# XuyangBai/D3Feat.pytorch

Hardware: AMD Instinct MI355X
Metric: fragment-pairs/sec (fwd+bwd) on 3DMatch-shaped pairs (higher is better)
Workload: dtype f32

## Files before the change

### d3feat.pytorch_amd/csrc/kpconv_dx_gather.hip

```cpp
#include "kpconv_tile.hpp"

namespace d3f {

void* kpconv_timing_open(int which, hipStream_t stream, int Nq, int Ns, int H, int Cin, int Cout, int K);
void kpconv_timing_close(void* rec, hipStream_t stream);

struct RevTest {
  const uint64_t* last_key;
  float sx, sy, sz;
  unsigned s;
  float r2;
};

template <int CV, bool HAS_NN>
__device__ __forceinline__ void dxg_table_chunk(int n, float qx, float qy, float qz, float nnv, uint64_t lk,
                                                const RevTest& rt, int Nq, int last_lane, int32_t* status,
                                                float4* scr4, float* scr1, __amdgpu_buffer_rsrc_t rs_g,
                                                unsigned row_bytes, unsigned col_off, float cx, float cy, float cz,
                                                float inv_extent, int lane, int lg, f32x4 (&acc)[CV]) {
  const float d2 = sqdist_exact(qx, qy, qz, rt.sx, rt.sy, rt.sz);
  const uint64_t key = ((uint64_t)__float_as_uint(d2) << 32) | rt.s;
  const bool in_r = rt.r2 <= 0.0f || d2 < rt.r2;
  const bool member = n < Nq && key <= lk && in_r;
  if (rt.r2 > 0.0f && status && lane == last_lane && n < Nq && d2 < rt.r2) atomicOr(status, D3F_ST_WIDE_OVERFLOW);
  const uint64_t m = __ballot(member);
  const int cnt = __popcll(m);
  if (cnt == 0) return;
  const int rank = __popcll(m & ((1ull << lane) - 1ull));
  if (member) {
    scr4[rank] = make_float4(qx - rt.sx, qy - rt.sy, qz - rt.sz, __int_as_float(n));
    scr1[rank] = HAS_NN ? 1.0f / nnv : 1.0f;
  }
  __builtin_amdgcn_fence(__ATOMIC_RELEASE, "wavefront");
  __builtin_amdgcn_wave_barrier();
  const bool mine = lane < cnt;
  const float4 c = scr4[mine ? lane : 0];
  const float inn = mine ? scr1[lane] : 0.0f;
  const int n_c = mine ? __float_as_int(c.w) : Nq;
  __builtin_amdgcn_wave_barrier();
  dxg_core_n<CV>((cnt + 15) >> 4, n_c, c.x, c.y, c.z, inn, rs_g, row_bytes, col_off, cx, cy, cz, inv_extent, lg, acc);
}

template <int CV, int NBW, int WK, bool HAS_NN>
__global__ __launch_bounds__(256) void kpconv_dx_gather_kernel(
    const float* __restrict__ s_pts, const float* __restrict__ q_pts, const int32_t* __restrict__ rev_ptr,
    const int32_t* __restrict__ rev_ent, const float* __restrict__ gout, const float* __restrict__ nn,
    const float* __restrict__ kp, const float* __restrict__ W, int Ns, int Nq, int Cin, int Cout, int K, float extent,
    float* __restrict__ gx, const uint64_t* __restrict__ last_key, int rev_width, float rev_r2,
    int32_t* __restrict__ status, unsigned long long* __restrict__ clk, const float4* __restrict__ rev_rel) {
  PhaseClock pc;
  pc.start(clk);
  constexpr int CC = 16 * CV;
  constexpr int WN = 4 / WK;
  extern __shared__ __attribute__((aligned(16))) float lds[];
  constexpr int RS = 16 * CC + 4;
  float* tile = lds;
  float4* scr4 = (float4*)(lds + 16 * RS) + (threadIdx.x >> 6) * 64;
  float* scr1 = lds + 16 * RS + 4 * 256 + (threadIdx.x >> 6) * 64;
  float* red = lds + 16 * RS + 5 * 256;

  const int lane = threadIdx.x & 63, wave = threadIdx.x >> 6;
  const int li = lane & 15, lg = lane >> 4;
  const int s0 = blockIdx.x * 16;
  float kx, ky, kz;
  load_kernel_point(kp, K, li, kx, ky, kz);
  const __amdgpu_buffer_rsrc_t rs_q = make_rsrc(q_pts, (unsigned)Nq * 12u);
  const __amdgpu_buffer_rsrc_t rs_nn = make_rsrc(HAS_NN ? nn : q_pts, (unsigned)Nq * 4u);
  const __amdgpu_buffer_rsrc_t rs_g = make_rsrc(gout, (unsigned)Nq * (unsigned)Cout * 4u);
  const float inv_extent = 1.0f / extent;
  const int wn = (WK == 1) ? wave : (WK == 2 ? (wave & 1) : 0);
  const int wk = (WK == 1) ? 0 : (WK == 2 ? (wave >> 1) : wave);
  constexpr int SLAB = 16 * NBW * WN;
  const int n_base = blockIdx.y * SLAB;

  constexpr int NACC = NBW == 1 ? 2 : 1;
  f32x4 acc2[NBW][NACC];
#pragma unroll
  for (int nb = 0; nb < NBW; ++nb)
#pragma unroll
    for (int a = 0; a < NACC; ++a) acc2[nb][a] = (f32x4){0.f, 0.f, 0.f, 0.f};
  if (WK > 1)
    for (int t = threadIdx.x; t < 16 * SLAB; t += 256) red[t] = 0.0f;

  const unsigned row_bytes = (unsigned)Cout * 4u;
  const int nchunks = Cout / CC;
  pc.lap(0);
  for (int ch = 0; ch < nchunks; ++ch) {
    const int cbase = ch * CC;
    const unsigned col_off = (unsigned)(cbase + li * CV) * 4u;
    if (rev_rel) {
      const int W = rev_width;
      float4 eA[4];
#pragma unroll
      for (int i = 0; i < 4; ++i) {
        const int s = s0 + wave * 4 + i;
        eA[i] = rev_rel[(size_t)min(s, Ns - 1) * W + min(lane, W - 1)];
        if (!(s < Ns && lane < W)) eA[i].w = __int_as_float(Nq);
      }
      if (clk) {
        asm volatile("s_waitcnt vmcnt(0)" ::: "memory");
        pc.lap(1);
      }
#pragma unroll 1
      for (int i = 0; i < 4; ++i) {
        const int s = s0 + wave * 4 + i;
        f32x4 acc[CV];
#pragma unroll
        for (int r = 0; r < CV; ++r) acc[r] = (f32x4){0.f, 0.f, 0.f, 0.f};
        if (s < Ns) {
          float4 e = eA[0];
          for (int c0 = 0; c0 < W; c0 += 64) {
            if (c0 > 0) {
              e = rev_rel[(size_t)s * W + min(c0 + lane, W - 1)];
              if (c0 + lane >= W) e.w = __int_as_float(Nq);
            }
            const int n = min(max(__float_as_int(e.w), 0), Nq);
            const int cnt = __popcll(__ballot(n < Nq));
            if (cnt == 0) break;
            if (HAS_NN)
              dxg_core_n<CV, true>((cnt + 15) >> 4, n, e.x, e.y, e.z, 0.0f, rs_g, row_bytes, col_off, -kx, -ky, -kz,
                                   inv_extent, lg, acc, Nq, rs_nn);
            else
              dxg_core_n<CV>((cnt + 15) >> 4, n, e.x, e.y, e.z, n < Nq ? 1.0f : 0.0f, rs_g, row_bytes, col_off, -kx, -ky,
                             -kz, inv_extent, lg, acc);
            if (cnt < 64) break;
          }
        }
        store_wf_tile<CV>(tile + (wave * 4 + i) * RS, li, lg, acc);
#pragma unroll
        for (int j = 0; j < 3; ++j) eA[j] = eA[j + 1];
      }
    } else if (last_key) {
      const int W = rev_width;
      const __amdgpu_buffer_rsrc_t rs_lk = make_rsrc(last_key, (unsigned)Nq * 8u);
      int nA[4], nB[4];
#pragma unroll
      for (int i = 0; i < 4; ++i) {
        const int s = s0 + wave * 4 + i;
        const size_t rb = (size_t)min(s, Ns - 1) * W;
        nA[i] = rev_ent[rb + min(lane, W - 1)];
        nB[i] = rev_ent[rb + min(64 + lane, W - 1)];
      }
#pragma unroll
      for (int i = 0; i < 4; ++i) {
        const bool row = s0 + wave * 4 + i < Ns;
        if (!(row && lane < W)) nA[i] = Nq;
        if (!(row && 64 + lane < W)) nB[i] = Nq;
      }
      float qx[4], qy[4], qz[4], nv[4] = {1.0f, 1.0f, 1.0f, 1.0f};
      int lklo[4], lkhi[4];
#pragma unroll
      for (int i = 0; i < 4; ++i) {
        nA[i] = min(max(nA[i], 0), Nq);
        nB[i] = min(max(nB[i], 0), Nq);
        const unsigned n = (unsigned)nA[i];
        qx[i] = __uint_as_float(__builtin_amdgcn_raw_buffer_load_b32(rs_q, n * 12u, 0, 0));
        qy[i] = __uint_as_float(__builtin_amdgcn_raw_buffer_load_b32(rs_q, n * 12u + 4u, 0, 0));
        qz[i] = __uint_as_float(__builtin_amdgcn_raw_buffer_load_b32(rs_q, n * 12u + 8u, 0, 0));
        if (HAS_NN) nv[i] = __uint_as_float(__builtin_amdgcn_raw_buffer_load_b32(rs_nn, n * 4u, 0, 0));
        const u32x2v k2 = __builtin_amdgcn_raw_buffer_load_b64(rs_lk, n * 8u, 0, 0);
        lklo[i] = (int)k2[0];
        lkhi[i] = (int)k2[1];
      }
      if (clk) {
        asm volatile("s_waitcnt vmcnt(0)" ::: "memory");
        pc.lap(1);
      }
#pragma unroll 1
      for (int i = 0; i < 4; ++i) {
        const int s = s0 + wave * 4 + i;
        f32x4 acc[CV];
#pragma unroll
        for (int r = 0; r < CV; ++r) acc[r] = (f32x4){0.f, 0.f, 0.f, 0.f};
        if (s < Ns) {
          const float sx = s_pts[3 * (size_t)s + 0], sy = s_pts[3 * (size_t)s + 1], sz = s_pts[3 * (size_t)s + 2];
          const float cx = -kx, cy = -ky, cz = -kz;
          const RevTest rt = {last_key, sx, sy, sz, (unsigned)s, rev_r2};
          int32_t* st = ch == 0 ? status : nullptr;
          const uint64_t lk_i = ((uint64_t)(unsigned)lkhi[0] << 32) | (unsigned)lklo[0];
          dxg_table_chunk<CV, HAS_NN>(nA[0], qx[0], qy[0], qz[0], nv[0], lk_i, rt, Nq, W <= 64 ? W - 1 : -1, st, scr4,
                                      scr1, rs_g, row_bytes, col_off, cx, cy, cz, inv_extent, lane, lg, acc);
          int nb = nB[0];
          for (int c0 = 64; c0 < W; c0 += 64) {
            if (c0 > 64) nb = (c0 + lane < W) ? min(max(rev_ent[(size_t)s * W + c0 + lane], 0), Nq) : Nq;
            if (__ballot(nb < Nq) == 0ull) break;
            const unsigned n = (unsigned)nb;
            const float bx = __uint_as_float(__builtin_amdgcn_raw_buffer_load_b32(rs_q, n * 12u, 0, 0));
            const float by = __uint_as_float(__builtin_amdgcn_raw_buffer_load_b32(rs_q, n * 12u + 4u, 0, 0));
            const float bz = __uint_as_float(__builtin_amdgcn_raw_buffer_load_b32(rs_q, n * 12u + 8u, 0, 0));
            const float bn =
                HAS_NN ? __uint_as_float(__builtin_amdgcn_raw_buffer_load_b32(rs_nn, n * 4u, 0, 0)) : 1.0f;
            const u32x2v k2 = __builtin_amdgcn_raw_buffer_load_b64(rs_lk, n * 8u, 0, 0);
            const int last = (W - 1 >= c0 && W - 1 < c0 + 64) ? W - 1 - c0 : -1;
            dxg_table_chunk<CV, HAS_NN>(nb, bx, by, bz, bn, ((uint64_t)k2[1] << 32) | k2[0], rt, Nq, last, st,
                                scr4, scr1, rs_g, row_bytes, col_off, cx, cy, cz, inv_extent, lane, lg, acc);
          }
        }
        store_wf_tile<CV>(tile + (wave * 4 + i) * RS, li, lg, acc);
#pragma unroll
        for (int j = 0; j < 3; ++j) {
          nA[j] = nA[j + 1]; nB[j] = nB[j + 1]; qx[j] = qx[j + 1]; qy[j] = qy[j + 1]; qz[j] = qz[j + 1];
          if (HAS_NN) nv[j] = nv[j + 1];
          lklo[j] = lklo[j + 1]; lkhi[j] = lkhi[j + 1];
        }
      }
    } else
#pragma unroll 1
    for (int i = 0; i < 4; ++i) {
      const int s = s0 + wave * 4 + i;
      f32x4 acc[CV];
#pragma unroll
      for (int r = 0; r < CV; ++r) acc[r] = (f32x4){0.f, 0.f, 0.f, 0.f};
      if (s < Ns) {
        const int beg = __builtin_amdgcn_readfirstlane(rev_ptr[s]);
        const int end = __builtin_amdgcn_readfirstlane(rev_ptr[s + 1]);
        const float sx = s_pts[3 * (size_t)s + 0], sy = s_pts[3 * (size_t)s + 1], sz = s_pts[3 * (size_t)s + 2];
        for (int c0 = beg; c0 < end; c0 += 64) {
          const int rem = min(end - c0, 64);
          const int n_raw = rev_ent[(size_t)c0 + min(lane, rem - 1)];
          const int n = lane < rem ? min(max(n_raw, 0), Nq) : Nq;
          const float qx = __uint_as_float(__builtin_amdgcn_raw_buffer_load_b32(rs_q, (unsigned)n * 12u, 0, 0));
          const float qy = __uint_as_float(__builtin_amdgcn_raw_buffer_load_b32(rs_q, (unsigned)n * 12u + 4u, 0, 0));
          const float qz = __uint_as_float(__builtin_amdgcn_raw_buffer_load_b32(rs_q, (unsigned)n * 12u + 8u, 0, 0));
          const float nnv =
              HAS_NN ? __uint_as_float(__builtin_amdgcn_raw_buffer_load_b32(rs_nn, (unsigned)n * 4u, 0, 0)) : 1.0f;
          const float inn = (lane < rem && n < Nq) ? (HAS_NN ? 1.0f / nnv : 1.0f) : 0.0f;
          dxg_core_n<CV>((rem + 15) >> 4, n, qx - sx, qy - sy, qz - sz, inn, rs_g, row_bytes, col_off, -kx, -ky, -kz,
                         inv_extent, lg, acc);
        }
      }
      store_wf_tile<CV>(tile + (wave * 4 + i) * RS, li, lg, acc);
    }
    pc.lap(2);
    __syncthreads();
    pc.lap(3);
    const int steps = (K * CC) >> 4;
    constexpr int BS = NBW >= 8 ? 1 : (NBW == 4 ? 2 : (NBW == 2 ? 4 : 8));
    for (int st0 = wk; st0 < steps; st0 += WK * BS) {
      float4 b[BS][NBW];
#pragma unroll
      for (int j = 0; j < BS; ++j) {
        const int sj = min(st0 + j * WK, steps - 1);
        const int kc0 = sj << 4;
        const int k = kc0 / CC, c0 = kc0 % CC;
#pragma unroll
        for (int nb = 0; nb < NBW; ++nb) {
          const int col = n_base + (wn + nb * WN) * 16 + li;
          b[j][nb] = *(const float4*)(W + ((size_t)k * Cin + col) * Cout + cbase + c0 + 4 * lg);
        }
      }
#pragma unroll
      for (int j = 0; j < BS; ++j) {
        const int sj = st0 + j * WK;
        if (sj < steps) {
          const float4 a = *(const float4*)(tile + li * RS + (sj << 4) + 4 * lg);
          const float av[4] = {a.x, a.y, a.z, a.w};
#pragma unroll
          for (int t = 0; t < 4; ++t)
#pragma unroll
            for (int nb = 0; nb < NBW; ++nb) {
              const float bv = t == 0 ? b[j][nb].x : (t == 1 ? b[j][nb].y : (t == 2 ? b[j][nb].z : b[j][nb].w));
              acc2[nb][t % NACC] = __builtin_amdgcn_mfma_f32_16x16x4f32(av[t], bv, acc2[nb][t % NACC], 0, 0, 0);
            }
        }
      }
    }
    pc.lap(4);
    __syncthreads();
  }
  f32x4 accf[NBW];
#pragma unroll
  for (int nb = 0; nb < NBW; ++nb) {
    accf[nb] = acc2[nb][0];
    if (NACC == 2) accf[nb] += acc2[nb][NACC - 1];
  }
  if (WK == 1) {
#pragma unroll
    for (int nb = 0; nb < NBW; ++nb) {
      const int col = n_base + (wn + nb * WN) * 16 + li;
#pragma unroll
      for (int r = 0; r < 4; ++r) {
        const int rowl = 4 * lg + r;
        if (s0 + rowl < Ns) gx[(size_t)(s0 + rowl) * Cin + col] = accf[nb][r];
      }
    }
  } else {
    for (int turn = 0; turn < WK; ++turn) {
      if (wk == turn) {
#pragma unroll
        for (int nb = 0; nb < NBW; ++nb) {
          const int col = (wn + nb * WN) * 16 + li;
#pragma unroll
          for (int r = 0; r < 4; ++r) red[(4 * lg + r) * SLAB + col] += accf[nb][r];
        }
      }
      __syncthreads();
    }
    for (int t = threadIdx.x; t < 16 * SLAB; t += 256) {
      const int rowl = t / SLAB, col = n_base + t % SLAB;
      if (s0 + rowl < Ns) gx[(size_t)(s0 + rowl) * Cin + col] = red[t];
    }
  }
  pc.lap(5);
  pc.done();
}

bool kpconv_dx_gather_supported(int Cin, int Cout, int K) {
  const bool cout_ok = (Cout == 16 || Cout == 32 || (Cout % 64 == 0 && Cout <= 512));
  const bool cin_ok = (Cin == 16 || Cin == 32 || Cin == 64 || Cin == 128 || Cin == 256 || Cin == 512);
  return cin_ok && cout_ok && K >= 1 && K <= 16;
}

template <int CV>
static int launch_dxg(const float* s_pts, const float* q_pts, const int32_t* rev_ptr, const int32_t* rev_ent,
                      const float* gout, const float* nn, const float* kp, const float* W, int Ns, int Nq, int Cin,
                      int Cout, int K, float extent, float* gx, const uint64_t* last_key, int rev_width, float rev_r2,
                      int32_t* status, const float4* rev_rel, hipStream_t stream) {
  const int tiles = cdiv(Ns, 16);
  constexpr int CC = 16 * CV;
  const size_t lds_base = sizeof(float) * (size_t)(16 * (16 * CC + 4) + 5 * 256);
  int slab = Cin;
  while (slab > 64 && (long long)tiles * (Cin / slab) < 512) slab >>= 1;
#define D3F_DXG(NBW, WK)                                                                                            \
  {                                                                                                                 \
    const size_t lds = lds_base + ((WK) > 1 ? sizeof(float) * 16 * (size_t)slab : 0);                               \
    dim3 grid(tiles, Cin / slab);                                                                                   \
    if (nn)                                                                                                         \
      kpconv_dx_gather_kernel<CV, NBW, WK, true><<<grid, 256, lds, stream>>>(                                       \
          s_pts, q_pts, rev_ptr, rev_ent, gout, nn, kp, W, Ns, Nq, Cin, Cout, K, extent, gx, last_key, rev_width,   \
          rev_r2, status, phase_clock_ptr(), rev_rel);                                                              \
    else                                                                                                            \
      kpconv_dx_gather_kernel<CV, NBW, WK, false><<<grid, 256, lds, stream>>>(                                      \
          s_pts, q_pts, rev_ptr, rev_ent, gout, nn, kp, W, Ns, Nq, Cin, Cout, K, extent, gx, last_key, rev_width,   \
          rev_r2, status, phase_clock_ptr(), rev_rel);                                                              \
  }
  void* timing = kpconv_timing_open(3, stream, Nq, Ns, 0, Cin, Cout, K);
  switch (slab) {
    case 16: D3F_DXG(1, 4) break;
    case 32: D3F_DXG(1, 2) break;
    case 64: D3F_DXG(1, 1) break;
    case 128: D3F_DXG(2, 1) break;
    case 256: D3F_DXG(4, 1) break;
    case 512: D3F_DXG(8, 1) break;
    default: return D3F_EINVAL;
  }
#undef D3F_DXG
  kpconv_timing_close(timing, stream);
  D3F_LAUNCH_CHECK();
  return D3F_OK;
}

}

extern "C" {

int d3f_kpconv_grad_input_gather_supported(int Cin, int Cout, int K) {
  return d3f::kpconv_dx_gather_supported(Cin, Cout, K) ? 1 : 0;
}

int d3f_kpconv_grad_input_gather(const float* q_pts, int Nq, const float* s_pts, int Ns, const int32_t* rev_ptr,
                                 const int32_t* rev_ent, const uint64_t* rev_last_key, int rev_width, float rev_radius,
                                 const float* rev_rel, const float* kernel_points, int K, const float* weights, int Cin,
                                 int Cout, float extent, const float* nn, const float* grad_out, float* grad_x,
                                 int32_t* status, void* stream) {
  if (!q_pts || !s_pts || !kernel_points || !weights || !grad_out || !grad_x || Nq < 0 || Ns < 0 ||
      !d3f::kpconv_dx_gather_supported(Cin, Cout, K) || !(extent > 0.0f))
    return D3F_EINVAL;
  if (rev_rel) {
    if (rev_ptr || rev_ent || rev_last_key || rev_width < 1 || ((uintptr_t)rev_rel & 15u)) return D3F_EINVAL;
  } else {
    if (!rev_ent || (rev_ptr != nullptr) == (rev_last_key != nullptr) || (!rev_ptr && rev_width < 1)) return D3F_EINVAL;
  }
  if ((double)Nq * Cout * 4.0 >= 4294967295.0 || (!rev_ptr && (double)Ns * rev_width >= 2147483647.0)) return D3F_EINVAL;
  if (Ns == 0) return D3F_OK;
  hipStream_t st = (hipStream_t)stream;
  const float rev_r2 = rev_radius > 0.0f ? rev_radius * rev_radius : 0.0f;
  const float4* rel = (const float4*)rev_rel;
  if (Cout == 16)
    return d3f::launch_dxg<1>(s_pts, q_pts, rev_ptr, rev_ent, grad_out, nn, kernel_points, weights, Ns, Nq, Cin, Cout, K, extent, grad_x, rev_last_key, rev_width, rev_r2, status, rel, st);
  if (Cout == 32)
    return d3f::launch_dxg<2>(s_pts, q_pts, rev_ptr, rev_ent, grad_out, nn, kernel_points, weights, Ns, Nq, Cin, Cout, K, extent, grad_x, rev_last_key, rev_width, rev_r2, status, rel, st);
  return d3f::launch_dxg<4>(s_pts, q_pts, rev_ptr, rev_ent, grad_out, nn, kernel_points, weights, Ns, Nq, Cin, Cout, K, extent, grad_x, rev_last_key, rev_width, rev_r2, status, rel, st);
}

}
```

### d3feat.pytorch_amd/csrc/kpconv_tile.hpp

```cpp
#pragma once
#include <type_traits>

#include "common.hpp"

namespace d3f {

typedef float f32x4 __attribute__((ext_vector_type(4)));
typedef unsigned u32x2v __attribute__((vector_size(8)));
typedef unsigned u32x4v __attribute__((vector_size(16)));

template <int CV>
struct VecT;
template <>
struct VecT<1> { typedef float type; };
template <>
struct VecT<2> { typedef float2 type; };
template <>
struct VecT<4> { typedef float4 type; };

template <int CV>
__device__ __forceinline__ float vget(const typename VecT<CV>::type& v, int r);
template <>
__device__ __forceinline__ float vget<1>(const float& v, int) { return v; }
template <>
__device__ __forceinline__ float vget<2>(const float2& v, int r) { return r == 0 ? v.x : v.y; }
template <>
__device__ __forceinline__ float vget<4>(const float4& v, int r) {
  return r == 0 ? v.x : (r == 1 ? v.y : (r == 2 ? v.z : v.w));
}

__device__ __forceinline__ __amdgpu_buffer_rsrc_t make_rsrc(const void* p, unsigned bytes) {
  return __builtin_amdgcn_make_buffer_rsrc(const_cast<void*>(p), 0, bytes, 0x00020000);
}
__device__ __forceinline__ float4 buf_load_f4(__amdgpu_buffer_rsrc_t r, unsigned off) {
  const u32x4v v = __builtin_amdgcn_raw_buffer_load_b128(r, off, 0, 0);
  return make_float4(__uint_as_float(v[0]), __uint_as_float(v[1]), __uint_as_float(v[2]), __uint_as_float(v[3]));
}
template <int CV>
__device__ __forceinline__ typename VecT<CV>::type buf_load_vec(__amdgpu_buffer_rsrc_t r, unsigned off);
template <>
__device__ __forceinline__ float buf_load_vec<1>(__amdgpu_buffer_rsrc_t r, unsigned off) {
  return __uint_as_float(__builtin_amdgcn_raw_buffer_load_b32(r, off, 0, 0));
}
template <>
__device__ __forceinline__ float2 buf_load_vec<2>(__amdgpu_buffer_rsrc_t r, unsigned off) {
  const u32x2v v = __builtin_amdgcn_raw_buffer_load_b64(r, off, 0, 0);
  return make_float2(__uint_as_float(v[0]), __uint_as_float(v[1]));
}
template <>
__device__ __forceinline__ float4 buf_load_vec<4>(__amdgpu_buffer_rsrc_t r, unsigned off) {
  return buf_load_f4(r, off);
}

constexpr float kFarKernelPoint = 1e18f;

__device__ __forceinline__ void load_kernel_point(const float* __restrict__ kp, int K, int li, float& kx, float& ky,
                                                  float& kz) {
  const float* p = kp + 3 * min(li, K - 1);
  const float x = p[0], y = p[1], z = p[2];
  const bool klive = li < K;
  kx = klive ? x : kFarKernelPoint;
  ky = klive ? y : kFarKernelPoint;
  kz = klive ? z : kFarKernelPoint;
}

__device__ __forceinline__ float kp_influence(const float4& sp, float cx, float cy, float cz, float inv_extent) {
  const float dx = sp.x - cx, dy = sp.y - cy, dz = sp.z - cz;
  const float d2 = fmaf(dz, dz, fmaf(dy, dy, dx * dx));
  return fmaxf(0.0f, fmaf(-__builtin_amdgcn_sqrtf(d2), inv_extent, 1.0f));
}

template <int CV, int NG>
struct QueryGather {
  float4 sp;
  typename VecT<CV>::type xv[NG];
};

template <int CV, int NSTEPS, typename Flush>
__device__ __forceinline__ void aggregate_wave_n(const int (&nall)[4], const float (&qx)[4], const float (&qy)[4],
                                                 const float (&qz)[4], float kx, float ky, float kz,
                                                 __amdgpu_buffer_rsrc_t rs_sp, __amdgpu_buffer_rsrc_t rs_x,
                                                 unsigned row_bytes, unsigned col_off, float inv_extent, int lg, int lane,
                                                 float* nn_lds, Flush&& flush) {
  constexpr int NG = 4 * NSTEPS;
  QueryGather<CV, NG> qg[1];
  auto gather = [&](QueryGather<CV, NG>& d, int nrow) {
    d.sp = buf_load_f4(rs_sp, (unsigned)nrow * 16u);
#pragma unroll
    for (int g = 0; g < NG; ++g) {
      const unsigned n = (unsigned)__shfl(nrow, 4 * g + lg, 64);
      d.xv[g] = buf_load_vec<CV>(rs_x, n * row_bytes + col_off);
    }
  };
#pragma unroll
  for (int i = 0; i < 4; ++i) {
    gather(qg[0], nall[i]);
    const QueryGather<CV, NG>& c = qg[0];
    if (nn_lds) {
      const float f = wave_sum(c.sp.w);
      if (lane == 0) nn_lds[i] = fmaxf(f, 1.0f);
    }
    const float rx = c.sp.x - qx[i], ry = c.sp.y - qy[i], rz = c.sp.z - qz[i];
    f32x4 acc[CV];
#pragma unroll
    for (int r = 0; r < CV; ++r) acc[r] = (f32x4){0.f, 0.f, 0.f, 0.f};
#pragma unroll
    for (int g = 0; g < NG; ++g) {
      float4 sp;
      sp.x = __shfl(rx, 4 * g + lg, 64);
      sp.y = __shfl(ry, 4 * g + lg, 64);
      sp.z = __shfl(rz, 4 * g + lg, 64);
      const float w = kp_influence(sp, kx, ky, kz, inv_extent);
#pragma unroll
      for (int r = 0; r < CV; ++r)
        acc[r] = __builtin_amdgcn_mfma_f32_16x16x4f32(w, vget<CV>(c.xv[g], r), acc[r], 0, 0, 0);
    }
    flush(i, acc);
  }
}

template <int DUMMY = 0>
__device__ __forceinline__ void load_wave_queries(const float* __restrict__ q_pts, const int32_t* __restrict__ idx,
                                                  int q_first, int Nq, int H, int Ns, int lane, int (&nall)[4],
                                                  float (&qx)[4], float (&qy)[4], float (&qz)[4]) {
  const int ls = min(lane, H - 1);
  int raw[4];
#pragma unroll
  for (int i = 0; i < 4; ++i) raw[i] = idx[(size_t)min(q_first + i, Nq - 1) * H + ls];
#pragma unroll
  for (int i = 0; i < 4; ++i) {
    const int qs = q_first + i < Nq ? q_first + i : 0;
    qx[i] = q_pts[3 * (size_t)qs + 0];
    qy[i] = q_pts[3 * (size_t)qs + 1];
    qz[i] = q_pts[3 * (size_t)qs + 2];
  }
#pragma unroll
  for (int i = 0; i < 4; ++i) {
    const int n = (q_first + i < Nq && lane < H) ? raw[i] : Ns;
    nall[i] = (int)min((unsigned)n, (unsigned)Ns);
  }
}

template <int CV, typename Flush>
__device__ __forceinline__ void aggregate_wave(const float* __restrict__ q_pts, const int32_t* __restrict__ idx,
                                               int q_first, int Nq, int H, int Ns, __amdgpu_buffer_rsrc_t rs_sp,
                                               __amdgpu_buffer_rsrc_t rs_x, int Cin, int cbase, float kx, float ky,
                                               float kz, float inv_extent, int lane, float* nn_lds, Flush&& flush) {
  const int li = lane & 15, lg = lane >> 4;
  const unsigned row_bytes = (unsigned)Cin * 4u;
  const unsigned col_off = (unsigned)(cbase + li * CV) * 4u;
  int nall[4];
  float qx[4], qy[4], qz[4];
  load_wave_queries(q_pts, idx, q_first, Nq, H, Ns, lane, nall, qx, qy, qz);
  const int nsteps = (H + 15) >> 4;
  if (nsteps == 3)
    aggregate_wave_n<CV, 3>(nall, qx, qy, qz, kx, ky, kz, rs_sp, rs_x, row_bytes, col_off, inv_extent, lg, lane, nn_lds,
                            flush);
  else if (nsteps == 2)
    aggregate_wave_n<CV, 2>(nall, qx, qy, qz, kx, ky, kz, rs_sp, rs_x, row_bytes, col_off, inv_extent, lg, lane, nn_lds,
                            flush);
  else if (nsteps == 4)
    aggregate_wave_n<CV, 4>(nall, qx, qy, qz, kx, ky, kz, rs_sp, rs_x, row_bytes, col_off, inv_extent, lg, lane, nn_lds,
                            flush);
  else
    aggregate_wave_n<CV, 1>(nall, qx, qy, qz, kx, ky, kz, rs_sp, rs_x, row_bytes, col_off, inv_extent, lg, lane, nn_lds,
                            flush);
}

template <int CV, int NSTEPS, typename Flush>
__device__ __forceinline__ void aggregate_wave_steps(const float* __restrict__ q_pts, const int32_t* __restrict__ idx,
                                                     int q_first, int Nq, int H, int Ns, __amdgpu_buffer_rsrc_t rs_sp,
                                                     __amdgpu_buffer_rsrc_t rs_x, int Cin, int cbase, float kx, float ky,
                                                     float kz, float inv_extent, int lane, float* nn_lds, Flush&& flush) {
  const int li = lane & 15, lg = lane >> 4;
  int nall[4];
  float qx[4], qy[4], qz[4];
  load_wave_queries(q_pts, idx, q_first, Nq, H, Ns, lane, nall, qx, qy, qz);
  aggregate_wave_n<CV, NSTEPS>(nall, qx, qy, qz, kx, ky, kz, rs_sp, rs_x, (unsigned)Cin * 4u,
                               (unsigned)(cbase + li * CV) * 4u, inv_extent, lg, lane, nn_lds, flush);
}

template <int CV, int NSTEPS, bool NN_GATHER>
__device__ __forceinline__ void dxg_core(int n_c, float qx, float qy, float qz, float inn, int Nq,
                                         __amdgpu_buffer_rsrc_t rs_nn, __amdgpu_buffer_rsrc_t rs_g, unsigned row_bytes, unsigned col_off, float cx,
                                         float cy, float cz, float inv_extent, int lg, f32x4 (&acc)[CV]) {
  constexpr int NG = 4 * NSTEPS;
  typename VecT<CV>::type xv[NG];
#pragma unroll
  for (int g = 0; g < NG; ++g) {
    const unsigned n = (unsigned)__shfl(n_c, 4 * g + lg, 64);
    xv[g] = buf_load_vec<CV>(rs_g, n * row_bytes + col_off);
  }
  if (NN_GATHER) {
    const float nv = __uint_as_float(__builtin_amdgcn_raw_buffer_load_b32(rs_nn, (unsigned)n_c * 4u, 0, 0));
    inn = n_c < Nq ? 1.0f / nv : 0.0f;
  }
#pragma unroll
  for (int g = 0; g < NG; ++g) {
    float4 sp;
    sp.x = __shfl(qx, 4 * g + lg, 64);
    sp.y = __shfl(qy, 4 * g + lg, 64);
    sp.z = __shfl(qz, 4 * g + lg, 64);
    sp.w = 0.0f;
    const float w = kp_influence(sp, cx, cy, cz, inv_extent) * __shfl(inn, 4 * g + lg, 64);
#pragma unroll
    for (int r = 0; r < CV; ++r)
      acc[r] = __builtin_amdgcn_mfma_f32_16x16x4f32(w, vget<CV>(xv[g], r), acc[r], 0, 0, 0);
  }
}

template <int CV, bool NN_GATHER = false>
__device__ __forceinline__ void dxg_core_n(int steps, int n_c, float qx, float qy, float qz, float inn,
                                           __amdgpu_buffer_rsrc_t rs_g, unsigned row_bytes, unsigned col_off, float cx,
                                           float cy, float cz, float inv_extent, int lg, f32x4 (&acc)[CV], int Nq = 0,
                                           __amdgpu_buffer_rsrc_t rs_nn = __amdgpu_buffer_rsrc_t()) {
  if (steps == 1) dxg_core<CV, 1, NN_GATHER>(n_c, qx, qy, qz, inn, Nq, rs_nn, rs_g, row_bytes, col_off, cx, cy, cz, inv_extent, lg, acc);
  else if (steps == 2) dxg_core<CV, 2, NN_GATHER>(n_c, qx, qy, qz, inn, Nq, rs_nn, rs_g, row_bytes, col_off, cx, cy, cz, inv_extent, lg, acc);
  else if (steps == 3) dxg_core<CV, 3, NN_GATHER>(n_c, qx, qy, qz, inn, Nq, rs_nn, rs_g, row_bytes, col_off, cx, cy, cz, inv_extent, lg, acc);
  else dxg_core<CV, 4, NN_GATHER>(n_c, qx, qy, qz, inn, Nq, rs_nn, rs_g, row_bytes, col_off, cx, cy, cz, inv_extent, lg, acc);
}

template <int CV>
__device__ __forceinline__ void store_wf_tile(float* __restrict__ dst_q, int li, int lg, const f32x4 (&acc)[CV]) {
  constexpr int CC = 16 * CV;
#pragma unroll
  for (int i = 0; i < 4; ++i) {
    float* dst = dst_q + (4 * lg + i) * CC + li * CV;
    if (CV == 1) dst[0] = acc[0][i];
    if (CV == 2) *(float2*)dst = make_float2(acc[0][i], acc[CV > 1 ? 1 : 0][i]);
    if (CV == 4)
      *(float4*)dst = make_float4(acc[0][i], acc[CV > 1 ? 1 : 0][i], acc[CV > 2 ? 2 : 0][i], acc[CV > 3 ? 3 : 0][i]);
  }
}

}
```

Measured before the change: 729.6.

## Pack four short reverse-neighbor rows into one gather pass in dx kernel

```diff
diff --git a/d3feat.pytorch_amd/csrc/kpconv_dx_gather.hip b/d3feat.pytorch_amd/csrc/kpconv_dx_gather.hip
--- a/d3feat.pytorch_amd/csrc/kpconv_dx_gather.hip
+++ b/d3feat.pytorch_amd/csrc/kpconv_dx_gather.hip
@@ -41,8 +41,20 @@
   dxg_core_n<CV>((cnt + 15) >> 4, n_c, c.x, c.y, c.z, inn, rs_g, row_bytes, col_off, cx, cy, cz, inv_extent, lg, acc);
 }
 
-template <int CV, int NBW, int WK, bool HAS_NN>
-__global__ __launch_bounds__(256) void kpconv_dx_gather_kernel(
+enum { DXG_EXACT = 0, DXG_SEARCH = 1, DXG_CSR = 2 };
+
+template <int CV, int FORM>
+constexpr int dxg_lds_floats() {
+  return 16 * (16 * 16 * CV + 4) + (FORM == DXG_SEARCH ? 5 * 256 : 0);
+}
+
+template <int CV, int NBW, int FORM>
+constexpr int dxg_min_waves() {
+  return FORM == DXG_EXACT ? (NBW == 1 ? 4 : (NBW == 2 ? 3 : 2)) : (FORM == DXG_SEARCH && CV == 1 && NBW == 4 ? 3 : 1);
+}
+
+template <int CV, int NBW, int WK, bool HAS_NN, int FORM>
+__global__ __launch_bounds__(256, (dxg_min_waves<CV, NBW, FORM>())) void kpconv_dx_gather_kernel(
     const float* __restrict__ s_pts, const float* __restrict__ q_pts, const int32_t* __restrict__ rev_ptr,
     const int32_t* __restrict__ rev_ent, const float* __restrict__ gout, const float* __restrict__ nn,
     const float* __restrict__ kp, const float* __restrict__ W, int Ns, int Nq, int Cin, int Cout, int K, float extent,
@@ -57,7 +69,7 @@
   float* tile = lds;
   float4* scr4 = (float4*)(lds + 16 * RS) + (threadIdx.x >> 6) * 64;
   float* scr1 = lds + 16 * RS + 4 * 256 + (threadIdx.x >> 6) * 64;
-  float* red = lds + 16 * RS + 5 * 256;
+  float* red = lds + dxg_lds_floats<CV, FORM>();
 
   const int lane = threadIdx.x & 63, wave = threadIdx.x >> 6;
   const int li = lane & 15, lg = lane >> 4;
@@ -88,7 +100,7 @@
   for (int ch = 0; ch < nchunks; ++ch) {
     const int cbase = ch * CC;
     const unsigned col_off = (unsigned)(cbase + li * CV) * 4u;
-    if (rev_rel) {
+    if (FORM == DXG_EXACT) {
       const int W = rev_width;
       float4 eA[4];
 #pragma unroll
@@ -101,36 +113,11 @@
         asm volatile("s_waitcnt vmcnt(0)" ::: "memory");
         pc.lap(1);
       }
-#pragma unroll 1
-      for (int i = 0; i < 4; ++i) {
-        const int s = s0 + wave * 4 + i;
-        f32x4 acc[CV];
-#pragma unroll
-        for (int r = 0; r < CV; ++r) acc[r] = (f32x4){0.f, 0.f, 0.f, 0.f};
-        if (s < Ns) {
-          float4 e = eA[0];
-          for (int c0 = 0; c0 < W; c0 += 64) {
-            if (c0 > 0) {
-              e = rev_rel[(size_t)s * W + min(c0 + lane, W - 1)];
-              if (c0 + lane >= W) e.w = __int_as_float(Nq);
-            }
-            const int n = min(max(__float_as_int(e.w), 0), Nq);
-            const int cnt = __popcll(__ballot(n < Nq));
-            if (cnt == 0) break;
-            if (HAS_NN)
-              dxg_core_n<CV, true>((cnt + 15) >> 4, n, e.x, e.y, e.z, 0.0f, rs_g, row_bytes, col_off, -kx, -ky, -kz,
-                                   inv_extent, lg, acc, Nq, rs_nn);
-            else
-              dxg_core_n<CV>((cnt + 15) >> 4, n, e.x, e.y, e.z, n < Nq ? 1.0f : 0.0f, rs_g, row_bytes, col_off, -kx, -ky,
-                             -kz, inv_extent, lg, acc);
-            if (cnt < 64) break;
-          }
-        }
-        store_wf_tile<CV>(tile + (wave * 4 + i) * RS, li, lg, acc);
-#pragma unroll
-        for (int j = 0; j < 3; ++j) eA[j] = eA[j + 1];
-      }
-    } else if (last_key) {
+      dxg_exact_rows<CV, HAS_NN, (CV <= 2)>(rev_rel, W, s0 + wave * 4, Ns, Nq, eA, rs_g, rs_nn, row_bytes, col_off, -kx,
+                                            -ky, -kz, inv_extent, lane, lg, [&](int i, const f32x4(&acc)[CV]) {
+                                              store_wf_tile<CV>(tile + (wave * 4 + i) * RS, li, lg, acc);
+                                            });
+    } else if (FORM == DXG_SEARCH) {
       const int W = rev_width;
       const __amdgpu_buffer_rsrc_t rs_lk = make_rsrc(last_key, (unsigned)Nq * 8u);
       int nA[4], nB[4];
@@ -317,22 +304,25 @@
                       int Cout, int K, float extent, float* gx, const uint64_t* last_key, int rev_width, float rev_r2,
                       int32_t* status, const float4* rev_rel, hipStream_t stream) {
   const int tiles = cdiv(Ns, 16);
-  constexpr int CC = 16 * CV;
-  const size_t lds_base = sizeof(float) * (size_t)(16 * (16 * CC + 4) + 5 * 256);
   int slab = Cin;
   while (slab > 64 && (long long)tiles * (Cin / slab) < 512) slab >>= 1;
-#define D3F_DXG(NBW, WK)                                                                                            \
+#define D3F_DXG_FORM(NBW, WK, NN, FORM)                                                                             \
   {                                                                                                                 \
-    const size_t lds = lds_base + ((WK) > 1 ? sizeof(float) * 16 * (size_t)slab : 0);                               \
-    dim3 grid(tiles, Cin / slab);                                                                                   \
-    if (nn)                                                                                                         \
-      kpconv_dx_gather_kernel<CV, NBW, WK, true><<<grid, 256, lds, stream>>>(                                       \
-          s_pts, q_pts, rev_ptr, rev_ent, gout, nn, kp, W, Ns, Nq, Cin, Cout, K, extent, gx, last_key, rev_width,   \
-          rev_r2, status, phase_clock_ptr(), rev_rel);                                                              \
-    else                                                                                                            \
-      kpconv_dx_gather_kernel<CV, NBW, WK, false><<<grid, 256, lds, stream>>>(                                      \
-          s_pts, q_pts, rev_ptr, rev_ent, gout, nn, kp, W, Ns, Nq, Cin, Cout, K, extent, gx, last_key, rev_width,   \
-          rev_r2, status, phase_clock_ptr(), rev_rel);                                                              \
+    const size_t lds = sizeof(float) * ((size_t)dxg_lds_floats<CV, FORM>() + ((WK) > 1 ? 16 * (size_t)slab : 0));   \
+    kpconv_dx_gather_kernel<CV, NBW, WK, NN, FORM><<<dim3(tiles, Cin / slab), 256, lds, stream>>>(                  \
+        s_pts, q_pts, rev_ptr, rev_ent, gout, nn, kp, W, Ns, Nq, Cin, Cout, K, extent, gx, last_key, rev_width,     \
+        rev_r2, status, phase_clock_ptr(), rev_rel);                                                                \
+  }
+#define D3F_DXG_NN(NBW, WK, NN)                               \
+  {                                                           \
+    if (rev_rel) D3F_DXG_FORM(NBW, WK, NN, DXG_EXACT)         \
+    else if (last_key) D3F_DXG_FORM(NBW, WK, NN, DXG_SEARCH)  \
+    else D3F_DXG_FORM(NBW, WK, NN, DXG_CSR)                   \
+  }
+#define D3F_DXG(NBW, WK)               \
+  {                                    \
+    if (nn) D3F_DXG_NN(NBW, WK, true)  \
+    else D3F_DXG_NN(NBW, WK, false)    \
   }
   void* timing = kpconv_timing_open(3, stream, Nq, Ns, 0, Cin, Cout, K);
   switch (slab) {
@@ -345,6 +335,8 @@
     default: return D3F_EINVAL;
   }
 #undef D3F_DXG
+#undef D3F_DXG_NN
+#undef D3F_DXG_FORM
   kpconv_timing_close(timing, stream);
   D3F_LAUNCH_CHECK();
   return D3F_OK;
diff --git a/d3feat.pytorch_amd/csrc/kpconv_tile.hpp b/d3feat.pytorch_amd/csrc/kpconv_tile.hpp
--- a/d3feat.pytorch_amd/csrc/kpconv_tile.hpp
+++ b/d3feat.pytorch_amd/csrc/kpconv_tile.hpp
@@ -181,22 +181,23 @@
 }
 
 template <int CV, int NSTEPS, bool NN_GATHER>
-__device__ __forceinline__ void dxg_core(int n_c, float qx, float qy, float qz, float inn, int Nq,
-                                         __amdgpu_buffer_rsrc_t rs_nn, __amdgpu_buffer_rsrc_t rs_g, unsigned row_bytes, unsigned col_off, float cx,
-                                         float cy, float cz, float inv_extent, int lg, f32x4 (&acc)[CV]) {
-  constexpr int NG = 4 * NSTEPS;
-  typename VecT<CV>::type xv[NG];
-#pragma unroll
-  for (int g = 0; g < NG; ++g) {
+__device__ __forceinline__ void dxg_request(int n_c, __amdgpu_buffer_rsrc_t rs_nn, __amdgpu_buffer_rsrc_t rs_g,
+                                            unsigned row_bytes, unsigned col_off, int lg,
+                                            typename VecT<CV>::type (&xv)[4 * NSTEPS], float& nv) {
+#pragma unroll
+  for (int g = 0; g < 4 * NSTEPS; ++g) {
     const unsigned n = (unsigned)__shfl(n_c, 4 * g + lg, 64);
     xv[g] = buf_load_vec<CV>(rs_g, n * row_bytes + col_off);
   }
-  if (NN_GATHER) {
-    const float nv = __uint_as_float(__builtin_amdgcn_raw_buffer_load_b32(rs_nn, (unsigned)n_c * 4u, 0, 0));
-    inn = n_c < Nq ? 1.0f / nv : 0.0f;
-  }
-#pragma unroll
-  for (int g = 0; g < NG; ++g) {
+  if (NN_GATHER) nv = __uint_as_float(__builtin_amdgcn_raw_buffer_load_b32(rs_nn, (unsigned)n_c * 4u, 0, 0));
+}
+
+template <int CV, int NSTEPS, int S0, int S1>
+__device__ __forceinline__ void dxg_fma(const typename VecT<CV>::type (&xv)[4 * NSTEPS], float qx, float qy, float qz,
+                                        float inn, float cx, float cy, float cz, float inv_extent, int lg,
+                                        f32x4 (&acc)[CV]) {
+#pragma unroll
+  for (int g = 4 * S0; g < 4 * S1; ++g) {
     float4 sp;
     sp.x = __shfl(qx, 4 * g + lg, 64);
     sp.y = __shfl(qy, 4 * g + lg, 64);
@@ -207,6 +208,17 @@
     for (int r = 0; r < CV; ++r)
       acc[r] = __builtin_amdgcn_mfma_f32_16x16x4f32(w, vget<CV>(xv[g], r), acc[r], 0, 0, 0);
   }
+}
+
+template <int CV, int NSTEPS, bool NN_GATHER>
+__device__ __forceinline__ void dxg_core(int n_c, float qx, float qy, float qz, float inn, int Nq,
+                                         __amdgpu_buffer_rsrc_t rs_nn, __amdgpu_buffer_rsrc_t rs_g, unsigned row_bytes, unsigned col_off, float cx,
+                                         float cy, float cz, float inv_extent, int lg, f32x4 (&acc)[CV]) {
+  typename VecT<CV>::type xv[4 * NSTEPS];
+  float nv = 1.0f;
+  dxg_request<CV, NSTEPS, NN_GATHER>(n_c, rs_nn, rs_g, row_bytes, col_off, lg, xv, nv);
+  if (NN_GATHER) inn = n_c < Nq ? 1.0f / nv : 0.0f;
+  dxg_fma<CV, NSTEPS, 0, NSTEPS>(xv, qx, qy, qz, inn, cx, cy, cz, inv_extent, lg, acc);
 }
 
 template <int CV, bool NN_GATHER = false>
@@ -220,6 +232,93 @@
   else dxg_core<CV, 4, NN_GATHER>(n_c, qx, qy, qz, inn, Nq, rs_nn, rs_g, row_bytes, col_off, cx, cy, cz, inv_extent, lg, acc);
 }
 
+__device__ __forceinline__ int dxg_entry_index(const float4& e, int Nq) { return min(max(__float_as_int(e.w), 0), Nq); }
+
+__device__ __forceinline__ int dxg_row_steps(const float4& e, int Nq) {
+  const int cnt = __popcll(__ballot(dxg_entry_index(e, Nq) < Nq));
+  return __builtin_amdgcn_readfirstlane((cnt + 15) >> 4);
+}
+
+template <int CV, int I, typename Flush>
+__device__ __forceinline__ void dxg_pack4_row(int steps, const typename VecT<CV>::type (&xv)[16], const float4& e,
+                                              float inn, float cx, float cy, float cz, float inv_extent, int lg,
+                                              Flush&& flush) {
+  f32x4 acc[CV];
+#pragma unroll
+  for (int r = 0; r < CV; ++r) acc[r] = (f32x4){0.f, 0.f, 0.f, 0.f};
+  if (steps >= 1) dxg_fma<CV, 4, I, I + 1>(xv, e.x, e.y, e.z, inn, cx, cy, cz, inv_extent, lg, acc);
+  flush(I, acc);
+}
+
+template <int CV, bool HAS_NN, typename Flush>
+__device__ __forceinline__ void dxg_pack4(const float4 (&eA)[4], const int (&st)[4], int Nq, __amdgpu_buffer_rsrc_t rs_g,
+                                          __amdgpu_buffer_rsrc_t rs_nn, unsigned row_bytes, unsigned col_off, float cx,
+                                          float cy, float cz, float inv_extent, int lane, int lg, Flush&& flush) {
+  float4 e = eA[0];
+#pragma unroll
+  for (int i = 1; i < 4; ++i) {
+    const int src = lane & 15;
+    const float4 t = make_float4(__shfl(eA[i].x, src, 64), __shfl(eA[i].y, src, 64), __shfl(eA[i].z, src, 64),
+                                 __shfl(eA[i].w, src, 64));
+    if ((lane >> 4) == i) e = t;
+  }
+  const int n = dxg_entry_index(e, Nq);
+  typename VecT<CV>::type xv[16];
+  float nv = 1.0f;
+  dxg_request<CV, 4, HAS_NN>(n, rs_nn, rs_g, row_bytes, col_off, lg, xv, nv);
+  const float inn = n < Nq ? (HAS_NN ? 1.0f / nv : 1.0f) : 0.0f;
+  dxg_pack4_row<CV, 0>(st[0], xv, e, inn, cx, cy, cz, inv_extent, lg, flush);
+  dxg_pack4_row<CV, 1>(st[1], xv, e, inn, cx, cy, cz, inv_extent, lg, flush);
+  dxg_pack4_row<CV, 2>(st[2], xv, e, inn, cx, cy, cz, inv_extent, lg, flush);
+  dxg_pack4_row<CV, 3>(st[3], xv, e, inn, cx, cy, cz, inv_extent, lg, flush);
+}
+
+template <int CV, bool HAS_NN, bool PACK4, typename Flush>
+__device__ __forceinline__ void dxg_exact_rows(const float4* __restrict__ rev_rel, int W, int s_first, int Ns, int Nq,
+                                               float4 (&eA)[4], __amdgpu_buffer_rsrc_t rs_g,
+                                               __amdgpu_buffer_rsrc_t rs_nn, unsigned row_bytes, unsigned col_off,
+                                               float cx, float cy, float cz, float inv_extent, int lane, int lg,
+                                               Flush&& flush) {
+  if (PACK4) {
+    int st[4];
+#pragma unroll
+    for (int i = 0; i < 4; ++i) st[i] = dxg_row_steps(eA[i], Nq);
+    if (max(max(st[0], st[1]), max(st[2], st[3])) == 1) {
+      dxg_pack4<CV, HAS_NN>(eA, st, Nq, rs_g, rs_nn, row_bytes, col_off, cx, cy, cz, inv_extent, lane, lg, flush);
+      return;
+    }
+  }
+#pragma unroll 1
+  for (int i = 0; i < 4; ++i) {
+    const int s = s_first + i;
+    f32x4 acc[CV];
+#pragma unroll
+    for (int c = 0; c < CV; ++c) acc[c] = (f32x4){0.f, 0.f, 0.f, 0.f};
+    if (s < Ns) {
+      float4 e = eA[0];
+      for (int c0 = 0; c0 < W; c0 += 64) {
+        if (c0 > 0) {
+          e = rev_rel[(size_t)s * W + min(c0 + lane, W - 1)];
+          if (c0 + lane >= W) e.w = __int_as_float(Nq);
+        }
+        const int n = dxg_entry_index(e, Nq);
+        const int cnt = __popcll(__ballot(n < Nq));
+        if (cnt == 0) break;
+        if (HAS_NN)
+          dxg_core_n<CV, true>((cnt + 15) >> 4, n, e.x, e.y, e.z, 0.0f, rs_g, row_bytes, col_off, cx, cy, cz, inv_extent,
+                               lg, acc, Nq, rs_nn);
+        else
+          dxg_core_n<CV>((cnt + 15) >> 4, n, e.x, e.y, e.z, n < Nq ? 1.0f : 0.0f, rs_g, row_bytes, col_off, cx, cy, cz,
+                         inv_extent, lg, acc);
+        if (cnt < 64) break;
+      }
+    }
+    flush(i, acc);
+#pragma unroll
+    for (int j = 0; j < 3; ++j) eA[j] = eA[j + 1];
+  }
+}
+
 template <int CV>
 __device__ __forceinline__ void store_wf_tile(float* __restrict__ dst_q, int li, int lg, const f32x4 (&acc)[CV]) {
   constexpr int CC = 16 * CV;
```

Result: no change. 729.7 (median of 2 runs) (+0.0%).
